# ShenhanQian/KGDet

Measured on AMD Instinct MI355X. Metric: training images/sec (whole node) KGDet R50-FPN 800x1333, higher is better.
Workload: dtype f32 (3 MFMA products per multiply on hi/lo-split operands -- fp16 parts forward, bf16 parts for gradients --, f32 accumulate); 1 GPU; KGDet R50-FPN train step, 2 img/GPU at 800x1333 (padded 800x1344), DeformConv fwd/bwd + focal/moment losses + grad-clip + Adam; no collective at dp1 (one rank: nothing to exchange); global_batch=2, parallelism=dp1

## Files before the change

### include/kgdet_hip.h

```cpp
#ifndef KGDET_HIP_H_
#define KGDET_HIP_H_

#include <stddef.h>
#include <stdint.h>

#ifdef __cplusplus
extern "C" {
#endif

#define KGDET_OK 0
#define KGDET_E_SHAPE 1
#define KGDET_E_WORKSPACE 2
#define KGDET_E_HIP 3
size_t kgdet_conv_packed_bytes(int32_t M, int32_t K, int32_t taps);
int kgdet_conv_pack(const float *w, int32_t O, int32_t C, int32_t taps, int32_t transpose, void *packed, void *stream);
int kgdet_conv_pack_fmt(const float *w, int32_t O, int32_t C, int32_t taps, int32_t transpose, void *packed,
                        int32_t operand_format, void *stream);
int kgdet_conv_pack_both_fmt(const float *w, int32_t O, int32_t C, int32_t taps, void *packed, void *packed_t,
                             int32_t forward_format, void *stream);
int kgdet_conv_apply_epilogue_fmt(const void *packed, const float *x, float *y, const float *bias, const float *residual,
                                  int32_t relu, int64_t B, int32_t M, int32_t K, int32_t H, int32_t W, int32_t taps,
                                  int32_t stride, int32_t operand_format, void *workspace, size_t workspace_bytes,
                                  void *stream);
int kgdet_conv_apply_gated_fmt(const void *packed, const float *x, float *y, const float *bias, const float *residual,
                               int32_t relu, const float *gate, int64_t B, int32_t M, int32_t K, int32_t H, int32_t W,
                               int32_t taps, int32_t stride, int32_t operand_format, void *workspace, size_t workspace_bytes,
                               void *stream);
int kgdet_stem_conv7x7_s2_fmt(const void *packed, const float *x, float *y, int64_t B, int32_t H, int32_t W,
                              int32_t operand_format, void *stream);
int kgdet_conv_pack_both(const float *w, int32_t O, int32_t C, int32_t taps, void *packed, void *packed_t, void *stream);
int64_t kgdet_conv_pack_blocks(int32_t O, int32_t C, int32_t taps);
int kgdet_conv_pack_multi(const int64_t *desc_dev, int32_t n, int64_t total_blocks, void *stream);
size_t kgdet_conv_apply_workspace_bytes(int64_t B, int32_t M, int32_t K, int32_t H, int32_t W, int32_t taps,
                                        int32_t stride);
int kgdet_conv_apply(const void *packed, const float *x, float *y, int64_t B, int32_t M, int32_t K, int32_t H, int32_t W,
                     int32_t taps, int32_t stride, void *workspace, size_t workspace_bytes, void *stream);
int kgdet_conv_apply_epilogue(const void *packed, const float *x, float *y, const float *bias, const float *residual,
                              int32_t relu, int64_t B, int32_t M, int32_t K, int32_t H, int32_t W, int32_t taps,
                              int32_t stride, void *workspace, size_t workspace_bytes, void *stream);
int kgdet_stem_conv7x7_s2(const void *packed, const float *x, float *y, int64_t B, int32_t H, int32_t W, void *stream);
int kgdet_conv3x3_s2_grad_input(const void *packed_t, const float *grad_y, float *grad_x, int64_t B, int32_t C, int32_t O,
                                int32_t Hin, int32_t Win, void *stream);
size_t kgdet_conv3x3_s2_grad_weight_workspace_bytes(int64_t B, int32_t O, int32_t C, int32_t H, int32_t W);
int kgdet_conv3x3_s2_grad_weight(const float *grad_y, const float *x, float *grad_w, int64_t B, int32_t O, int32_t C, int32_t H,
                                 int32_t W, void *workspace, size_t workspace_bytes, void *stream);
size_t kgdet_conv1x1_grad_weight_workspace_bytes(int64_t B, int32_t O, int32_t C, int64_t HW);
int kgdet_conv1x1_grad_weight(const float *grad_y, const float *x, float *grad_w, int64_t B, int32_t O, int32_t C,
                              int64_t HW, void *workspace, size_t workspace_bytes, void *stream);
size_t kgdet_conv3x3_grad_weight_workspace_bytes(int64_t B, int32_t O, int32_t C, int32_t H, int32_t W);
int kgdet_conv3x3_grad_weight(const float *grad_y, const float *x, float *grad_w, int64_t B, int32_t O, int32_t C,
                              int32_t H, int32_t W, void *workspace, size_t workspace_bytes, void *stream);

int kgdet_bn_act_forward(const float *x, const float *gamma, const float *beta, const float *mean, const float *var,
                         float eps, const float *residual, float *y, int64_t N, int32_t C, int64_t HW, int32_t relu,
                         void *stream);
int32_t kgdet_bn_act_partials(int64_t N, int32_t C, int64_t HW);
int kgdet_bn_act_backward(const float *grad_y, const float *x, const float *y, const float *gamma, const float *beta,
                          const float *mean, const float *var, float eps, int32_t has_residual, int32_t relu,
                          float *grad_x, float *grad_residual, float *partial, float *sums, int64_t N, int32_t C,
                          int64_t HW, void *stream);
int kgdet_conv1x1_nhwc_residual(const void *x, const void *weight, const float *bias, const void *residual, void *out,
                                int64_t M, int32_t K, int32_t N, int32_t relu, void *stream);
int kgdet_conv1x1_nhwc_residual_in(const void *x, const float *in_bias, const void *weight, const float *bias,
                                   const void *residual, void *out, int64_t M, int32_t K, int32_t N, int32_t relu,
                                   void *stream);
int kgdet_bn_fold_backward(const float *grad_z, const float *z, int32_t relu, float *g, float *partial, int64_t N, int32_t C,
                           int64_t HW, void *stream);
int kgdet_bn_fold_finish(const float *partial, int32_t P, const float *w, float *G , const float *s,
                         const float *mean, const float *var, float eps, float *grad_beta ,
                         float *grad_gamma , int32_t O, int32_t CK, void *stream);
int kgdet_conv1x1_grad_weight_fold(const float *grad_y, const float *x, float *grad_w, int64_t B, int32_t O, int32_t C,
                                   int64_t HW, void *workspace, size_t workspace_bytes, const float *w, const float *s,
                                   const float *mean, const float *var, float eps, const float *bn_partial, int32_t P,
                                   float *grad_beta , float *grad_gamma , void *stream);
int kgdet_conv3x3_grad_weight_fold(const float *grad_y, const float *x, float *grad_w, int64_t B, int32_t O, int32_t C,
                                   int32_t H, int32_t W, void *workspace, size_t workspace_bytes, const float *w,
                                   const float *s, const float *mean, const float *var, float eps, const float *bn_partial,
                                   int32_t P, float *grad_beta , float *grad_gamma , void *stream);
int kgdet_bn_relu_maxpool(const float *x, const float *gamma, const float *beta, const float *mean, const float *var,
                          float eps, float *y, int64_t N, int32_t C, int32_t H, int32_t W, void *stream);

int kgdet_bias_act(void *x, const float *bias, const void *residual, int64_t N, int32_t C, int64_t HW, int32_t dtype,
                   int32_t relu, int32_t channels_last, void *stream);
int kgdet_bias_relu_maxpool_nhwc(const void *x, const float *bias, void *y, int64_t N, int32_t C, int32_t H, int32_t W,
                                 int32_t dtype, void *stream);

#define KGDET_E_UNSUPPORTED 4
#define KGDET_E_PARTIAL 5

const char *kgdet_last_error(void);
int kgdet_version(void);
int kgdet_device_cu_count(void);

#define KGDET_OPT_EXACT_BACKWARD 0
#define KGDET_OPT_FWD_COLUMN_WAVE 1
#define KGDET_OPT_WGRAD_STREAMK 2
#define KGDET_OPT_BWD_PHASE 3
#define KGDET_OPT_COUNT 4
int kgdet_set_option(int32_t option, int32_t value);

typedef struct kgdet_dcn_shape {
  int32_t N, C, H, W;
  int32_t O, kh, kw;
  int32_t stride_h, stride_w, pad_h, pad_w, dil_h, dil_w;
  int32_t groups, deformable_groups;
  int32_t out_channel_offset, out_channels_total;
} kgdet_dcn_shape;

#define KGDET_DCN_RELU 1u
#define KGDET_DCN_BF16 2u
#define KGDET_DCN_EXACT_FP32 4u

int kgdet_dcn_output_size(const kgdet_dcn_shape *s, int32_t *Ho, int32_t *Wo);

size_t kgdet_dcn_packed_weight_bytes(const kgdet_dcn_shape *s);
size_t kgdet_dcn_workspace_bytes(const kgdet_dcn_shape *s);

int kgdet_dcn_pack_weight(const kgdet_dcn_shape *s, const float *weight, float *packed, void *stream);
int kgdet_dcn_pack_weight_multi(int32_t n, const kgdet_dcn_shape *const *shapes, const float *const *weights,
                                float *const *packeds, void *stream);
int kgdet_dcn_pack_weight_images(int32_t n, const kgdet_dcn_shape *const *shapes, const float *const *weights,
                                 float *const *packeds, uint32_t images, void *stream);
int32_t kgdet_dcn_split_path_complete(const kgdet_dcn_shape *shape);
int kgdet_dcn_unpack_weight_grad(const kgdet_dcn_shape *s, const float *packed, float *grad_weight,
                                 int accumulate, void *stream);

int kgdet_deform_conv_forward(const kgdet_dcn_shape *s, const float *input, const float *offset,
                              const float *mask , const float *packed_weight,
                              const float *bias , float *output, uint32_t flags,
                              void *workspace, size_t workspace_bytes, void *stream);

size_t kgdet_dcn_group_workspace_bytes(int32_t n, const kgdet_dcn_shape *const *shapes);

int kgdet_deform_conv_forward_grouped(int32_t n, const kgdet_dcn_shape *const *shapes, const float *const *inputs,
                                      const float *const *offsets, const float *const *masks ,
                                      const float *const *packed_weights, const float *const *biases ,
                                      float *const *outputs, uint32_t flags, void *workspace,
                                      size_t workspace_bytes, void *stream);

int kgdet_deform_conv_grad_input(const kgdet_dcn_shape *s, const float *offset, const float *mask ,
                                 const float *packed_weight, const float *grad_output, float *grad_input,
                                 uint32_t flags, void *workspace, size_t workspace_bytes, void *stream);

int kgdet_deform_conv_grad_offset(const kgdet_dcn_shape *s, const float *input, const float *offset,
                                  const float *packed_weight, const float *grad_output, float *grad_offset,
                                  uint32_t flags, void *workspace, size_t workspace_bytes, void *stream);

int kgdet_deform_conv_backward_input_grouped(int32_t n, const kgdet_dcn_shape *const *shapes, const float *const *inputs,
                                             const float *const *offsets, const float *const *packed_weights,
                                             const float *const *grad_outputs, float *const *grad_inputs,
                                             float *const *grad_offsets, void *workspace, size_t workspace_bytes,
// ... 188 lines not shown
```

### kgdet_amd/csrc/dense_forward.hip

```cpp
#include "dense_common.h"

namespace kgdet {

__global__ __launch_bounds__(256) void conv1x1_pack(const float *__restrict__ w, int O, int C, int T, int transpose,
                                                    unsigned char *__restrict__ img, unsigned char *__restrict__ img_t,
                                                    int f16_forward) {
  if (gridDim.y == 2) {
    transpose = blockIdx.y;
    img = blockIdx.y ? img_t : img;
  }
  const bool f16 = f16_forward && !transpose;
  f16_saturate_on();
  const int M = transpose ? C : O, K = transpose ? O : C;
  const int k16s = (K + kTK - 1) / kTK;
  const long long total = (long long)((M + kTM - 1) / kTM) * k16s * T * 2 * kTM;
  for (long long i = blockIdx.x * 256LL + threadIdx.x; i < total; i += gridDim.x * 256LL) {
    const int row = (int)(i % kTM);
    const int khalf = (int)((i / kTM) & 1);
    const long long st = i / (2 * kTM);
    const int t = (int)(st % T);
    const int k16 = (int)((st / T) % k16s), mt = (int)(st / ((long long)T * k16s));
    const int m = mt * kTM + row, k0 = k16 * kTK + khalf * 8;
    float v[8];
#pragma unroll
// ... 48 lines not shown
        const f32x4 u = src[q];
        r[4 * q] = u[0]; r[4 * q + 1] = u[1]; r[4 * q + 2] = u[2]; r[4 * q + 3] = u[3];
      }
      const float sc9 = (scale && m < M) ? scale[m] : 1.0f;
#pragma unroll
      for (int t = 0; t < 9; ++t) {
        float v[8];
#pragma unroll
        for (int j = 0; j < 8; ++j) v[j] = m < M ? r[j * 9 + t] * sc9 : 0.0f;
        bf16x8 hi8, lo8;
        if (f16_forward) {
#pragma unroll
          for (int j = 0; j < 8; ++j) v[j] *= kF16WeightScale;
          split8_t<true>(v, hi8, lo8);
        } else {
          split8(v, hi8, lo8);
        }
        unsigned char *dst = img + (s2 * 9 + t) * kStage + khalf * (kTM * 16) + row * 16;
        *reinterpret_cast<bf16x8 *>(dst) = hi8;
        *reinterpret_cast<bf16x8 *>(dst + kPart) = lo8;
      }
      continue;
    }
    if (i >= total) continue;
    const int row = (int)(i % kTM);
    const int khalf = (int)((i / kTM) & 1);
    const long long st = i / (2 * kTM);
    const int t = (int)(st % T);
    const int k16 = (int)((st / T) % k16s), mt = (int)(st / ((long long)T * k16s));
    const int m = mt * kTM + row, k0 = k16 * kTK + khalf * 8;
    float v[8];
#pragma unroll
    for (int j = 0; j < 8; ++j) {
      const long long o = transpose ? k0 + j : m, ch = transpose ? m : k0 + j;
      v[j] = (m < M && k0 + j < K) ? w[(o * C + ch) * T + (transpose ? T - 1 - t : t)] : 0.0f;
      if (scale && m < M && k0 + j < K) v[j] *= scale[o];
    }
    bf16x8 hi8, lo8;
    if (f16_forward && !transpose) {
#pragma unroll
      for (int j = 0; j < 8; ++j) v[j] *= kF16WeightScale;
      split8_t<true>(v, hi8, lo8);
    } else {
      split8(v, hi8, lo8);
    }
    unsigned char *dst = img + st * kStage + khalf * (kTM * 16) + row * 16;
    *reinterpret_cast<bf16x8 *>(dst) = hi8;
    *reinterpret_cast<bf16x8 *>(dst + kPart) = lo8;
  }
}

constexpr int kPF = 4;

template <int TAPS, int NW = 4, bool F16 = false>
__global__ __launch_bounds__(128 * NW) void conv_nn(const unsigned char *__restrict__ img,
                                                      const float *__restrict__ x, float *__restrict__ y, int M, int K,
                                                      int H, int W, int n_mt, int n_nt, int tiles, int ksplit,
                                                      long long part_stride, int Hin, int Win, int stride,
                                                      const float *__restrict__ bias,
                                                      const float *__restrict__ residual, int relu,
    const float *__restrict__ gate = nullptr) {
  constexpr int TN = 32 * NW, kPartB = 2 * TN * 16, kBuf = kStage + 2 * kPartB;
  __shared__ __attribute__((aligned(16))) unsigned char smem[2 * kBuf];
  if constexpr (F16) f16_saturate_on();
  const int unit = xcd_tile(blockIdx.x, tiles * ksplit);
  if (unit >= tiles * ksplit) return;
  const int part = unit % ksplit, tile = unit / ksplit;
  const int tid = threadIdx.x, lane = tid & 63, wave = tid >> 6, wm = wave & 1, wn = wave >> 1;
  const int n_local = tid % TN, kq = tid / TN;
  const int N = H * W;
  const int S = TAPS * ((K + kTK - 1) / kTK), per = (S + ksplit - 1) / ksplit;
  const int s_begin = part * per, s_end = max(s_begin, min(S, s_begin + per));
  const int stages = s_end - s_begin;
  struct Regs {
    f32x4 a;
    float v[4];
    unsigned live;
  };
  const int mt = tile % n_mt, nt = (tile / n_mt) % n_nt, b = tile / (n_mt * n_nt);
  const int n0 = nt * TN;
  const int p = min(n0 + n_local, N - 1);
  unsigned ok = 1u;
  if (TAPS == 9) {
    const int h = (p / W) * stride, w = (p - (p / W) * W) * stride;
    ok = 0u;
#pragma unroll
    for (int t = 0; t < 9; ++t) {
      const int hh = h + t / 3 - 1, ww = w + t % 3 - 1;
      ok |= (hh >= 0 && hh < Hin && ww >= 0 && ww < Win) ? (1u << t) : 0u;
    }
  }
  const int Nin = Hin * Win;
  const int pin = stride == 1 ? p : (p / W) * stride * Win + (p - (p / W) * W) * stride;
  const float *xb = x + (long long)b * K * Nin + pin;
  const unsigned char *ai = img + (long long)mt * S * kStage + (tid & 511) * 16;

  f32x16 acc[2];
#pragma unroll
  for (int i = 0; i < 2; ++i)
#pragma unroll
    for (int r = 0; r < 16; ++r) acc[i][r] = 0.0f;

  auto issue = [&](int s, Regs &R) {
    const int sc = s_begin + min(s, stages - 1);
    R.a = *reinterpret_cast<const f32x4 *>(ai + (long long)sc * kStage);
    const int c16 = sc / TAPS, t = sc - c16 * TAPS;
    int shift = 0;
    R.live = 1u;
    if (TAPS == 9) {
      R.live = (ok >> t) & 1u;
      shift = R.live ? (t / 3 - 1) * Win + (t % 3 - 1) : 0;
    }
    const float *xp = xb + (long long)(c16 * kTK + kq * 4) * Nin + shift;
    if (TAPS == 1 && (K & (kTK - 1)) && c16 == K / kTK) {
#pragma unroll
      for (int j = 0; j < 4; ++j) R.v[j] = xb[(long long)min(c16 * kTK + kq * 4 + j, K - 1) * Nin];
    } else {
#pragma unroll
      for (int j = 0; j < 4; ++j) R.v[j] = xp[(long long)j * Nin];
    }
  };
  auto commit = [&](int buf, const Regs &R) {
    unsigned char *As = smem + buf * kBuf, *Bs = As + kStage;
    *reinterpret_cast<f32x4 *>(As + (tid & 511) * 16) = R.a;
    uint2 hi, lo;
    split_pair_t<F16>(R.live ? R.v[0] : 0.0f, R.live ? R.v[1] : 0.0f, hi.x, lo.x);
    split_pair_t<F16>(R.live ? R.v[2] : 0.0f, R.live ? R.v[3] : 0.0f, hi.y, lo.y);
    unsigned char *dst = Bs + (kq >> 1) * (TN * 16) + n_local * 16 + (kq & 1) * 8;
    *reinterpret_cast<uint2 *>(dst) = hi;
    *reinterpret_cast<uint2 *>(dst + kPartB) = lo;
  };
  auto multiply = [&](int buf) {
    const unsigned char *A = smem + buf * kBuf + (lane >> 5) * (kTM * 16) + (wm * 64 + (lane & 31)) * 16;
    const unsigned char *Bp = smem + buf * kBuf + kStage + (lane >> 5) * (TN * 16) + (wn * 32 + (lane & 31)) * 16;
    bf16x8 a[2][2], bb[2];
#pragma unroll
    for (int pt = 0; pt < 2; ++pt) {
      a[pt][0] = *reinterpret_cast<const bf16x8 *>(A + pt * kPart);
      a[pt][1] = *reinterpret_cast<const bf16x8 *>(A + pt * kPart + 32 * 16);
      bb[pt] = *reinterpret_cast<const bf16x8 *>(Bp + pt * kPartB);
    }
#pragma unroll
    for (int mi = 0; mi < 2; ++mi) {
      acc[mi] = mfma_t<F16>(a[1][mi], bb[0], acc[mi]);
      acc[mi] = mfma_t<F16>(a[0][mi], bb[1], acc[mi]);
      acc[mi] = mfma_t<F16>(a[0][mi], bb[0], acc[mi]);
    }
  };
  {
    Regs R[kPF];
#pragma unroll
    for (int i = 0; i < kPF; ++i) issue(i, R[i]);
    commit(0, R[0]);
    const int full = stages / kPF * kPF;
    for (int s0 = 0; s0 < full; s0 += kPF) {
#pragma unroll
      for (int u = 0; u < kPF; ++u) {
        const int s = s0 + u;
        __syncthreads();
        issue(s + kPF, R[u]);
        multiply(s & 1);
        commit((s + 1) & 1, R[(u + 1) % kPF]);
      }
    }
#pragma unroll
    for (int u = 0; u < kPF - 1; ++u) {
      const int s = full + u;
      if (s < stages) {
        __syncthreads();
        multiply(s & 1);
        if (s + 1 < stages) commit((s + 1) & 1, R[u + 1]);
      }
    }
  }

  float *yb = y + (long long)part * part_stride + (long long)b * M * N;
  const int n = n0 + wn * 32 + (lane & 31);
  if constexpr (F16) {
#pragma unroll
    for (int mi = 0; mi < 2; ++mi)
#pragma unroll
      for (int r = 0; r < 16; ++r) acc[mi][r] *= 1.0f / kF16WeightScale;
  }
  if (bias || residual) {
    const int nc = min(n, N - 1);
    float add[2][16];
#pragma unroll
    for (int mi = 0; mi < 2; ++mi)
#pragma unroll
      for (int r = 0; r < 16; ++r) {
        const int m = min(mt * kTM + wm * 64 + mi * 32 + (r & 3) + 8 * (r >> 2) + 4 * (lane >> 5), M - 1);
        float v = bias ? bias[m] : 0.0f;
        if (residual) v += residual[((long long)b * M + m) * N + nc];
        add[mi][r] = v;
      }
#pragma unroll
    for (int mi = 0; mi < 2; ++mi)
#pragma unroll
      for (int r = 0; r < 16; ++r) acc[mi][r] += add[mi][r];
  }
  if (gate) {
    const int nc = min(n, N - 1);
    float gv[2][16];
#pragma unroll
    for (int mi = 0; mi < 2; ++mi)
#pragma unroll
      for (int r = 0; r < 16; ++r) {
        const int m = min(mt * kTM + wm * 64 + mi * 32 + (r & 3) + 8 * (r >> 2) + 4 * (lane >> 5), M - 1);
        gv[mi][r] = gate[((long long)b * M + m) * N + nc];
      }
#pragma unroll
    for (int mi = 0; mi < 2; ++mi)
#pragma unroll
      for (int r = 0; r < 16; ++r) acc[mi][r] = gv[mi][r] > 0.0f ? acc[mi][r] : 0.0f;
  }
#pragma unroll
  for (int mi = 0; mi < 2; ++mi)
#pragma unroll
    for (int r = 0; r < 16; ++r) {
      const int m = mt * kTM + wm * 64 + mi * 32 + (r & 3) + 8 * (r >> 2) + 4 * (lane >> 5);
      if (m < M && n < N) yb[(long long)m * N + n] = relu ? fmaxf(acc[mi][r], 0.0f) : acc[mi][r];
    }
}

constexpr int kPatchMax = 256;
constexpr int kPatchPart = 2 * kPatchMax * 16;
constexpr int kPatchBuf = 2 * kPatchPart;
template <int WAVES, int NB, bool F16 = false>
__global__ __launch_bounds__(64 * WAVES) void conv3x3_patch4(const unsigned char *__restrict__ img,
                                                             const float *__restrict__ x, float *__restrict__ y, int M,
                                                             int K, int H, int W, int n_mt, int tiles_x, int n_nt,
                                                             int tiles, int ksplit, long long part_stride, int TX, int TY,
                                                             const float *__restrict__ bias,
                                                             const float *__restrict__ residual, int relu,
    const float *__restrict__ gate = nullptr) {
  __shared__ __attribute__((aligned(16))) unsigned char smem[2 * kPatchBuf];
  if constexpr (F16) f16_saturate_on();
  constexpr int HALVES = 4 / WAVES, THREADS = 64 * WAVES, PXT = kPatchMax / THREADS;
  const int unit0 = xcd_tile(blockIdx.x, tiles * ksplit * HALVES);
  if (unit0 >= tiles * ksplit * HALVES) return;
  const int half = unit0 % HALVES, unit = unit0 / HALVES;
  const int part = unit % ksplit, tile = unit / ksplit;
  const int tid = threadIdx.x, lane = tid & 63, wave = (tid >> 6) + half * WAVES;
  const int N = H * W;
  const int chunks_all = K / kTK, per = (chunks_all + ksplit - 1) / ksplit;
  const int c_begin = part * per, c_end = max(c_begin, min(chunks_all, c_begin + per));
  const int chunks = c_end - c_begin, stages = chunks * 9;
  const int mt = tile % n_mt, nt = (tile / n_mt) % n_nt, b = tile / (n_mt * n_nt);
  const int y0 = (nt / tiles_x) * TY, x0 = (nt % tiles_x) * TX;
  const int PW = TX + 2, PP = PW * (TY + 2);

  if (mt * kTM + half * 64 >= M) return;
  bool p_live[PXT];
  int p_off[PXT];
#pragma unroll
  for (int i = 0; i < PXT; ++i) {
    const int pp = tid + i * THREADS;
    const int ppy = pp / PW, ppx = pp - ppy * PW;
    const int iy = y0 - 1 + ppy, ix = x0 - 1 + ppx;
    p_live[i] = pp < PP && iy >= 0 && iy < H && ix >= 0 && ix < W;
    p_off[i] = p_live[i] ? iy * W + ix : 0;
  }
  const float *xb = x + (long long)b * K * N;
  unsigned char *b_dst = smem + tid * 16;

  int b_rd[NB], o_n[NB];
  bool o_live[NB];
#pragma unroll
  for (int nb = 0; nb < NB; ++nb) {
    const int qq = nb * 32 + (lane & 31), q = min(qq, TX * TY - 1);
    const int py = q / TX, px = q - py * TX;
    b_rd[nb] = ((lane >> 5) * kPatchMax + py * PW + px) * 16;
    o_live[nb] = qq < TX * TY && y0 + py < H && x0 + px < W;
// ... 303 lines not shown

__global__ __launch_bounds__(256) void conv1x1_sum_epilogue(const float *__restrict__ parts, float *__restrict__ out,
                                                            long long n, long long stride, int count,
                                                            const float *__restrict__ bias, const float *__restrict__ residual,
                                                            int relu, int M, long long HW,
                                                            const float *__restrict__ gate = nullptr) {
  for (long long i = (blockIdx.x * 256LL + threadIdx.x) * 2; i < n; i += gridDim.x * 512LL) {
    f32x2 s = {0.0f, 0.0f};
    int k = 0;
    for (; k + 4 <= count; k += 4) {
      f32x2 v[4];
#pragma unroll
      for (int e = 0; e < 4; ++e) v[e] = *reinterpret_cast<const f32x2 *>(parts + (long long)(k + e) * stride + i);
#pragma unroll
      for (int e = 0; e < 4; ++e) s += v[e];
    }
    for (; k < count; ++k) s += *reinterpret_cast<const f32x2 *>(parts + (long long)k * stride + i);
    if (bias) {
      const float b = bias[(i / HW) % M];
      s[0] += b; s[1] += b;
    }
    if (residual) s += *reinterpret_cast<const f32x2 *>(residual + i);
    if (relu) { s[0] = fmaxf(s[0], 0.0f); s[1] = fmaxf(s[1], 0.0f); }
    if (gate) {
      const f32x2 gv = *reinterpret_cast<const f32x2 *>(gate + i);
      s[0] = gv[0] > 0.0f ? s[0] : 0.0f; s[1] = gv[1] > 0.0f ? s[1] : 0.0f;
    }
    *reinterpret_cast<f32x2 *>(out + i) = s;
  }
}

namespace {

long long pack_items(int M, int K, int taps) { return (long long)ceil_div(M, kTM) * ceil_div(K, kTK) * taps * 2 * kTM; }
long long pack_both_blocks(int O, int C, int taps) {
  const long long t0 = pack_items(O, C, taps), t1 = pack_items(C, O, taps);
  return ((t0 > t1 ? t0 : t1) + 255) / 256;
}

template <typename Kernel, typename... Args>
void launch_fmt(bool f16, Kernel bf16_kernel, Kernel f16_kernel, unsigned grid, unsigned block, void *stream, Args... args) {
  hipLaunchKernelGGL(f16 ? f16_kernel : bf16_kernel, dim3(grid), dim3(block), 0, (hipStream_t)stream, args...);
}

int nn_ksplit(long long tiles, int stages) {
  if (tiles >= 200) return 1;
  int k = (int)((384 + tiles - 1) / tiles);
  const int most = stages / 8;
  if (k > most) k = most;
  if (k > 8) k = 8;
  return k < 1 ? 1 : k;
}

struct NNPlan {
  bool patch;
  int TX, TY, NB, NW, tiles_x, n_nt, ks;
  long long tiles;
};
NNPlan plan_nn(long long B, int M, int K, int H, int W, int taps, int stride) {
  NNPlan p;
  const int Ho = (H + stride - 1) / stride, Wo = (W + stride - 1) / stride;
  const int n_mt = (M + kTM - 1) / kTM;
  p.patch = taps == 9 && stride == 1;
  p.TX = p.TY = p.tiles_x = 0;
  p.NB = p.NW = 4;
  p.n_nt = (int)(((long long)Ho * Wo + kTN - 1) / kTN);
  if (p.patch) {
    long long best = -1;
    for (int cap = 128; cap <= (M > 64 ? 160 : 128); cap += 32)
      for (int tx = 8; tx <= 126 && tx <= (W + 7) / 8 * 8; ++tx) {
        const int ty = cap / tx;
        if (ty < 1 || (tx + 2) * (ty + 2) > kPatchMax) continue;
        const long long n = (long long)((H + ty - 1) / ty) * ((W + tx - 1) / tx);
        const long long units = n * n_mt * B;
        const long long rounds = units <= 256 ? 256 : units <= 512 ? 512 : units;
        const long long cost = (rounds * (cap / 32)) * 4096 + n * 8 + (cap == 160) * 4 + ((tx + 2) * (ty + 2) > 230);
        if (best < 0 || cost < best) { best = cost; p.TX = tx; p.TY = ty; p.NB = cap / 32; }
      }
    static const int force_tx = env_int("KGDET_CONV_TX", 0);
    if (force_tx > 0 && (force_tx + 2) * (128 / force_tx + 2) <= kPatchMax) { p.TX = force_tx; p.TY = 128 / force_tx; p.NB = 4; }
    p.tiles_x = (W + p.TX - 1) / p.TX;
    p.n_nt = p.tiles_x * ((H + p.TY - 1) / p.TY);
  } else {
    static const int force_nw = env_int("KGDET_CONV_NW", 0);
    const long long hw = (long long)Ho * Wo;
    const long long u4 = (long long)n_mt * ((hw + 127) / 128) * B, u5 = (long long)n_mt * ((hw + 159) / 160) * B;
    const long long c4 = ((u4 + 255) / 256) * 4, c5 = ((u5 + 255) / 256) * 5;
    if (force_nw == 5 || (force_nw == 0 && u4 >= 200 && u5 >= 200 && c5 * 10 <= c4 * 9)) {
      p.NW = 5;
      p.n_nt = (int)((hw + 159) / 160);
    }
  }
  p.tiles = (long long)n_mt * p.n_nt * B;
  p.ks = nn_ksplit(p.tiles, taps * ((K + kTK - 1) / kTK));
  if (p.patch && p.tiles < 200) {
    const int chunks = K / kTK;
    double best = 1e30;
    p.ks = 1;
    for (int ks = 1; ks <= 8 && ks * 2 <= chunks; ++ks) {
      const double out_mb = (double)B * M * Ho * Wo * 4e-6;
      const double cost = (double)((p.tiles * ks + 255) / 256) * ((chunks + ks - 1) / ks) + 0.114 * out_mb * ks;
      if (cost < best) { best = cost; p.ks = ks; }
    }
  }
  static const int force_ks = env_int("KGDET_CONV_KS", 0);
  if (force_ks > 0) p.ks = force_ks;
  return p;
}

}

}

using namespace kgdet;

extern "C" size_t kgdet_conv_packed_bytes(int32_t M, int32_t K, int32_t taps) {
  if (M <= 0 || K <= 0 || (taps == 9 && K % kTK) || (taps != 1 && taps != 9)) return 0;
  return (size_t)pack_items(M, K, taps) * 32;
}

extern "C" int kgdet_conv_pack_fmt(const float *w, int32_t O, int32_t C, int32_t taps, int32_t transpose, void *packed,
                                   int32_t operand_format, void *stream) {
  const int M = transpose ? C : O, K = transpose ? O : C;
  KGDET_CHECK_SHAPE(taps == 1 || taps == 9, "taps must be 1 (1x1) or 9 (3x3)");
  KGDET_CHECK_SHAPE(O > 0 && C > 0 && (taps == 1 || K % kTK == 0), "reduction length %d is not a multiple of 16", K);
  KGDET_CHECK_SHAPE(w && packed, "null pointer");
  const long long blocks = (pack_items(M, K, taps) + 255) / 256;
  hipLaunchKernelGGL(conv1x1_pack, dim3((unsigned)(blocks > 65535 ? 65535 : blocks)), dim3(256), 0, (hipStream_t)stream, w,
                     O, C, taps, transpose, (unsigned char *)packed, (unsigned char *)nullptr, operand_format == 1 ? 1 : 0);
  KGDET_CHECK_LAUNCH("conv_pack");
  return KGDET_OK;
}

extern "C" int kgdet_conv_pack(const float *w, int32_t O, int32_t C, int32_t taps, int32_t transpose, void *packed,
                               void *stream) {
  return kgdet_conv_pack_fmt(w, O, C, taps, transpose, packed, 0, stream);
}

extern "C" int kgdet_conv_pack_both_fmt(const float *w, int32_t O, int32_t C, int32_t taps, void *packed, void *packed_t,
                                        int32_t forward_format, void *stream) {
  KGDET_CHECK_SHAPE(taps == 1 || taps == 9, "taps must be 1 (1x1) or 9 (3x3)");
  KGDET_CHECK_SHAPE(O > 0 && C > 0 && (taps == 1 || (O % kTK == 0 && C % kTK == 0)), "O and C must be multiples of 16");
  KGDET_CHECK_SHAPE(w && packed && packed_t, "null pointer");
  const long long blocks = pack_both_blocks(O, C, taps);
  hipLaunchKernelGGL(conv1x1_pack, dim3((unsigned)(blocks > 32768 ? 32768 : blocks), 2), dim3(256), 0,
                     (hipStream_t)stream, w, O, C, taps, 0, (unsigned char *)packed, (unsigned char *)packed_t,
                     forward_format == 1 ? 1 : 0);
  KGDET_CHECK_LAUNCH("conv_pack_both");
  return KGDET_OK;
}

extern "C" int kgdet_conv_pack_both(const float *w, int32_t O, int32_t C, int32_t taps, void *packed, void *packed_t,
                                    void *stream) {
  return kgdet_conv_pack_both_fmt(w, O, C, taps, packed, packed_t, 0, stream);
}

extern "C" int64_t kgdet_conv_pack_blocks(int32_t O, int32_t C, int32_t taps) {
  if (O <= 0 || C <= 0 || (taps == 9 && (O % kTK || C % kTK)) || (taps != 1 && taps != 9)) return 0;
  return pack_both_blocks(O, C, taps);
}

extern "C" int kgdet_conv_pack_multi(const int64_t *desc_dev, int32_t n, int64_t total_blocks, void *stream) {
  KGDET_CHECK_SHAPE(desc_dev && n > 0 && total_blocks > 0 && total_blocks < (1LL << 31), "bad descriptor table");
  hipLaunchKernelGGL(conv1x1_pack_multi, dim3((unsigned)total_blocks), dim3(256), 0, (hipStream_t)stream,
                     (const long long *)desc_dev, n);
  KGDET_CHECK_LAUNCH("conv_pack_multi");
  return KGDET_OK;
}

extern "C" size_t kgdet_conv_apply_workspace_bytes(int64_t B, int32_t M, int32_t K, int32_t H, int32_t W,
                                                    int32_t taps, int32_t stride) {
  if (B <= 0 || M <= 0 || K <= 0 || H <= 0 || W <= 0 || (taps == 9 && K % kTK) || stride < 1 || stride > 2) return 0;
  const long long HW = (long long)((H + stride - 1) / stride) * ((W + stride - 1) / stride);
  const int ks = plan_nn(B, M, K, H, W, taps, stride).ks;
  return ks > 1 ? (size_t)ks * B * M * HW * sizeof(float) : 0;
}

extern "C" int kgdet_conv_apply_epilogue_fmt(const void *packed, const float *x, float *y, const float *bias,
                                             const float *residual, int32_t relu, int64_t B, int32_t M, int32_t K,
                                             int32_t H, int32_t W, int32_t taps, int32_t stride, int32_t operand_format,
                                             void *workspace, size_t workspace_bytes, void *stream) {
  return kgdet_conv_apply_gated_fmt(packed, x, y, bias, residual, relu, nullptr, B, M, K, H, W, taps, stride, operand_format,
                                    workspace, workspace_bytes, stream);
}

extern "C" int kgdet_conv_apply_gated_fmt(const void *packed, const float *x, float *y, const float *bias,
                                          const float *residual, int32_t relu, const float *gate, int64_t B, int32_t M,
                                          int32_t K, int32_t H, int32_t W, int32_t taps, int32_t stride,
                                          int32_t operand_format, void *workspace, size_t workspace_bytes, void *stream) {
  const bool f16 = operand_format == 1;
  KGDET_CHECK_SHAPE(B >= 0 && M > 0 && K > 0 && H >= 0 && W >= 0 && (long long)H * W < (1LL << 30), "bad sizes");
  KGDET_CHECK_SHAPE(taps == 1 || taps == 9, "taps must be 1 (1x1) or 9 (3x3)");
  KGDET_CHECK_SHAPE(stride == 1 || stride == 2, "stride must be 1 or 2");
  KGDET_CHECK_SHAPE(taps == 1 || K % kTK == 0, "reduction length %d is not a multiple of 16", K);
  const int Ho = (H + stride - 1) / stride, Wo = (W + stride - 1) / stride;
  const long long HW = (long long)Ho * Wo;
  if (B * HW == 0) return KGDET_OK;
  KGDET_CHECK_SHAPE(packed && x && y, "null pointer");
  const NNPlan plan = plan_nn(B, M, K, H, W, taps, stride);
  const int n_mt = (M + kTM - 1) / kTM, n_nt = plan.n_nt;
  const long long tiles = plan.tiles;
  KGDET_CHECK_SHAPE(tiles < (1LL << 28), "too many tiles");
  const int ks = plan.ks;
  const long long part_stride = B * M * HW;
  if (ks > 1) {
    KGDET_CHECK_SHAPE(workspace && workspace_bytes >= (size_t)ks * part_stride * sizeof(float), "workspace too small");
    KGDET_CHECK_SHAPE(part_stride % 2 == 0, "B*M*Ho*Wo must be even");
    KGDET_CHECK_SHAPE(!gate || HW % 2 == 0, "a gated K-split convolution needs an even pixel count");
  }
  const unsigned grid = (unsigned)((tiles * ks + 7) / 8) * 8;
  float *dst = ks > 1 ? (float *)workspace : y;
  const float *k_bias = ks > 1 ? nullptr : bias, *k_residual = ks > 1 ? nullptr : residual, *k_gate = ks > 1 ? nullptr : gate;
  const int k_relu = ks > 1 ? 0 : relu;
  const unsigned char *img = (const unsigned char *)packed;
  if (plan.patch) {
    static const int force_halves = env_int("KGDET_CONV_HALVES", -1);
    const bool halves = force_halves >= 0 ? force_halves != 0 : ((ks == 1 && tiles > 256 && tiles < 400) || M <= 64);
    auto launch = [&](auto bf16_kernel, auto f16_kernel, unsigned g, unsigned threads) {
      launch_fmt(f16, bf16_kernel, f16_kernel, g, threads, stream, img, x, dst, M, K, H, W, n_mt, plan.tiles_x, n_nt, (int)tiles,
                 ks, part_stride, plan.TX, plan.TY, k_bias, k_residual, k_relu, k_gate);
    };
    if (plan.NB == 5)
      launch(conv3x3_patch4<4, 5, false>, conv3x3_patch4<4, 5, true>, grid, 256);
    else if (halves)
      launch(conv3x3_patch4<2, 4, false>, conv3x3_patch4<2, 4, true>, (unsigned)((tiles * ks * 2 + 7) / 8) * 8, 128);
    else
      launch(conv3x3_patch4<4, 4, false>, conv3x3_patch4<4, 4, true>, grid, 256);
  } else {
    auto launch = [&](auto bf16_kernel, auto f16_kernel, unsigned threads) {
      launch_fmt(f16, bf16_kernel, f16_kernel, grid, threads, stream, img, x, dst, M, K, Ho, Wo, n_mt, n_nt, (int)tiles, ks,
                 part_stride, H, W, stride, k_bias, k_residual, k_relu, k_gate);
    };
    if (taps == 1 && plan.NW == 5)
      launch(conv_nn<1, 5, false>, conv_nn<1, 5, true>, 640);
    else if (taps == 1)
      launch(conv_nn<1, 4, false>, conv_nn<1, 4, true>, 512);
    else if (plan.NW == 5)
      launch(conv_nn<9, 5, false>, conv_nn<9, 5, true>, 640);
    else
      launch(conv_nn<9, 4, false>, conv_nn<9, 4, true>, 512);
  }
  KGDET_CHECK_LAUNCH("conv_nn");
  if (ks > 1) {
    const long long blocks = (part_stride / 2 + 255) / 256;
    if ((bias || residual || relu || gate) && HW % 2 == 0)
      hipLaunchKernelGGL(conv1x1_sum_epilogue, dim3((unsigned)(blocks > 2048 ? 2048 : blocks)), dim3(256), 0,
                         (hipStream_t)stream, (const float *)workspace, y, part_stride, part_stride, ks, bias, residual, relu,
                         M, (long long)HW, gate);
    else
      hipLaunchKernelGGL(conv1x1_sum, dim3((unsigned)(blocks > 2048 ? 2048 : blocks)), dim3(256), 0, (hipStream_t)stream,
                         (const float *)workspace, y, part_stride, part_stride, ks);
    KGDET_CHECK_LAUNCH("conv1x1_sum");
    if ((bias || residual || relu) && HW % 2 != 0) return kgdet_bias_act(y, bias, residual, B, M, HW, 0, relu, 0, stream);
  }
  return KGDET_OK;
}

extern "C" int kgdet_conv_apply_epilogue(const void *packed, const float *x, float *y, const float *bias,
                                         const float *residual, int32_t relu, int64_t B, int32_t M, int32_t K,
                                         int32_t H, int32_t W, int32_t taps, int32_t stride, void *workspace,
                                         size_t workspace_bytes, void *stream) {
  return kgdet_conv_apply_epilogue_fmt(packed, x, y, bias, residual, relu, B, M, K, H, W, taps, stride, 0, workspace,
                                       workspace_bytes, stream);
}

extern "C" int kgdet_conv3x3_s2_grad_input(const void *packed_t, const float *grad_y, float *grad_x, int64_t B, int32_t C,
                                           int32_t O, int32_t Hin, int32_t Win, void *stream) {
  KGDET_CHECK_SHAPE(B >= 0 && C > 0 && O > 0 && Hin > 0 && Win > 0 && O % kTK == 0, "bad sizes (O must be a multiple of 16)");
  if (B == 0) return KGDET_OK;
  KGDET_CHECK_SHAPE(packed_t && grad_y && grad_x, "null pointer");
  const int H = (Hin + 1) / 2, W = (Win + 1) / 2;
  int TX = 0, TY = 0;
  long long best = -1;
  for (int tx = 8; tx <= 64; ++tx) {
    const int ty = 64 / tx;
    if (ty < 1 || (tx + 2) * (ty + 2) > kPatchMax) continue;
    const long long n = (long long)((H + ty - 1) / ty) * ((W + tx - 1) / tx);
    const long long cost = n * 1024 + (tx + 2) * (ty + 2);
    if (best < 0 || cost < best) { best = cost; TX = tx; TY = ty; }
  }
  const int n_mt = (C + kTM - 1) / kTM, tiles_x = (W + TX - 1) / TX, n_nt = tiles_x * ((H + TY - 1) / TY);
  const long long tiles = (long long)n_mt * n_nt * B;
  KGDET_CHECK_SHAPE(tiles < (1LL << 28), "too many tiles");
  hipLaunchKernelGGL(conv3x3_s2_grad_input, dim3((unsigned)((tiles + 7) / 8 * 8)), dim3(256), 0, (hipStream_t)stream,
                     (const unsigned char *)packed_t, grad_y, grad_x, C, O, H, W, Hin, Win, n_mt, tiles_x, n_nt, (int)tiles, TX, TY);
  KGDET_CHECK_LAUNCH("conv3x3_s2_grad_input");
// ... 29 lines not shown
```

Measured before the change: 186.4 img/s.

## Add 64-row conv_nn workgroups and cost-model choice of row tile and K-split

Templates the forward conv_nn kernel on a 64-row output tile, where four waves are laid out along the pixels. The planner gains an occupancy- and cost-based rule that picks 64-row tiles and a matching K-split for small tile counts (under 200 tiles), for both the generic and the patch 3x3 paths. The aim is to fill more of the 256 CUs on low-parallelism layers where 128-row tiles leave most CUs idle. In exchange the A operand is re-read per half-tile and the choice rests on hand-tuned constants. A plan query API and option knobs are also added.

```diff
diff --git a/include/kgdet_hip.h b/include/kgdet_hip.h
--- a/include/kgdet_hip.h
+++ b/include/kgdet_hip.h
@@ -33,6 +33,12 @@
 int kgdet_conv_pack_multi(const int64_t *desc_dev, int32_t n, int64_t total_blocks, void *stream);
 size_t kgdet_conv_apply_workspace_bytes(int64_t B, int32_t M, int32_t K, int32_t H, int32_t W, int32_t taps,
                                         int32_t stride);
+typedef struct kgdet_conv_plan {
+  int32_t rows, pixel_tile, tile_w, tile_h, ks, patch;
+  int64_t workgroups;
+} kgdet_conv_plan;
+int kgdet_conv_apply_plan(int64_t B, int32_t M, int32_t K, int32_t H, int32_t W, int32_t taps, int32_t stride,
+                          kgdet_conv_plan *plan);
 int kgdet_conv_apply(const void *packed, const float *x, float *y, int64_t B, int32_t M, int32_t K, int32_t H, int32_t W,
                      int32_t taps, int32_t stride, void *workspace, size_t workspace_bytes, void *stream);
 int kgdet_conv_apply_epilogue(const void *packed, const float *x, float *y, const float *bias, const float *residual,
@@ -96,7 +102,9 @@
 #define KGDET_OPT_FWD_COLUMN_WAVE 1
 #define KGDET_OPT_WGRAD_STREAMK 2
 #define KGDET_OPT_BWD_PHASE 3
-#define KGDET_OPT_COUNT 4
+#define KGDET_OPT_CONV_ROWS 4
+#define KGDET_OPT_CONV_KS 5
+#define KGDET_OPT_COUNT 6
 int kgdet_set_option(int32_t option, int32_t value);
 
 typedef struct kgdet_dcn_shape {
diff --git a/kgdet_amd/csrc/dense_forward.hip b/kgdet_amd/csrc/dense_forward.hip
--- a/kgdet_amd/csrc/dense_forward.hip
+++ b/kgdet_amd/csrc/dense_forward.hip
@@ -124,21 +124,28 @@
 
 constexpr int kPF = 4;
 
-template <int TAPS, int NW = 4, bool F16 = false>
-__global__ __launch_bounds__(128 * NW) void conv_nn(const unsigned char *__restrict__ img,
+constexpr int nn_threads(int rows, int nw) { return rows * nw; }
+constexpr int nn_lds_bytes(int rows, int nw) { return 2 * (rows * 64 + 2 * (2 * 32 * nw * 16)); }
+template <int TAPS, int NW = 4, bool F16 = false, int ROWS = 128>
+__global__ __launch_bounds__(nn_threads(ROWS, NW)) void conv_nn(const unsigned char *__restrict__ img,
                                                       const float *__restrict__ x, float *__restrict__ y, int M, int K,
                                                       int H, int W, int n_mt, int n_nt, int tiles, int ksplit,
                                                       long long part_stride, int Hin, int Win, int stride,
                                                       const float *__restrict__ bias,
                                                       const float *__restrict__ residual, int relu,
     const float *__restrict__ gate = nullptr) {
-  constexpr int TN = 32 * NW, kPartB = 2 * TN * 16, kBuf = kStage + 2 * kPartB;
+  static_assert(ROWS == 128 || (ROWS == 64 && NW == 4), "64-row workgroups: four waves along the pixels only");
+  constexpr int WM = ROWS / 64, THREADS = nn_threads(ROWS, NW);
+  constexpr int kPartA = 2 * ROWS * 16, kStageA = 2 * kPartA;
+  constexpr int TN = 32 * NW, kPartB = 2 * TN * 16, kBuf = kStageA + 2 * kPartB;
+  constexpr int CPT = kTK * TN / THREADS, QPT = CPT / 4;
+  static_assert(2 * kBuf == nn_lds_bytes(ROWS, NW), "plan_nn counts co-resident workgroups from nn_lds_bytes");
   __shared__ __attribute__((aligned(16))) unsigned char smem[2 * kBuf];
   if constexpr (F16) f16_saturate_on();
   const int unit = xcd_tile(blockIdx.x, tiles * ksplit);
   if (unit >= tiles * ksplit) return;
   const int part = unit % ksplit, tile = unit / ksplit;
-  const int tid = threadIdx.x, lane = tid & 63, wave = tid >> 6, wm = wave & 1, wn = wave >> 1;
+  const int tid = threadIdx.x, lane = tid & 63, wave = tid >> 6, wm = wave % WM, wn = wave / WM;
   const int n_local = tid % TN, kq = tid / TN;
   const int N = H * W;
   const int S = TAPS * ((K + kTK - 1) / kTK), per = (S + ksplit - 1) / ksplit;
@@ -146,10 +153,11 @@
   const int stages = s_end - s_begin;
   struct Regs {
     f32x4 a;
-    float v[4];
+    float v[CPT];
     unsigned live;
   };
   const int mt = tile % n_mt, nt = (tile / n_mt) % n_nt, b = tile / (n_mt * n_nt);
+  const int row0 = mt * ROWS;
   const int n0 = nt * TN;
   const int p = min(n0 + n_local, N - 1);
   unsigned ok = 1u;
@@ -165,7 +173,9 @@
   const int Nin = Hin * Win;
   const int pin = stride == 1 ? p : (p / W) * stride * Win + (p - (p / W) * W) * stride;
   const float *xb = x + (long long)b * K * Nin + pin;
-  const unsigned char *ai = img + (long long)mt * S * kStage + (tid & 511) * 16;
+  const int a_src = ROWS == 128 ? (tid & 511) * 16 : (tid >> 6) * (kTM * 16) + ((mt & 1) * 64 + (tid & 63)) * 16;
+  const int a_dst = ROWS == 128 ? (tid & 511) * 16 : tid * 16;
+  const unsigned char *ai = img + (long long)(row0 / kTM) * S * kStage + a_src;
 
   f32x16 acc[2];
 #pragma unroll
@@ -183,33 +193,37 @@
       R.live = (ok >> t) & 1u;
       shift = R.live ? (t / 3 - 1) * Win + (t % 3 - 1) : 0;
     }
-    const float *xp = xb + (long long)(c16 * kTK + kq * 4) * Nin + shift;
+    const float *xp = xb + (long long)(c16 * kTK + kq * CPT) * Nin + shift;
     if (TAPS == 1 && (K & (kTK - 1)) && c16 == K / kTK) {
 #pragma unroll
-      for (int j = 0; j < 4; ++j) R.v[j] = xb[(long long)min(c16 * kTK + kq * 4 + j, K - 1) * Nin];
+      for (int j = 0; j < CPT; ++j) R.v[j] = xb[(long long)min(c16 * kTK + kq * CPT + j, K - 1) * Nin];
     } else {
 #pragma unroll
-      for (int j = 0; j < 4; ++j) R.v[j] = xp[(long long)j * Nin];
+      for (int j = 0; j < CPT; ++j) R.v[j] = xp[(long long)j * Nin];
     }
   };
   auto commit = [&](int buf, const Regs &R) {
-    unsigned char *As = smem + buf * kBuf, *Bs = As + kStage;
-    *reinterpret_cast<f32x4 *>(As + (tid & 511) * 16) = R.a;
-    uint2 hi, lo;
-    split_pair_t<F16>(R.live ? R.v[0] : 0.0f, R.live ? R.v[1] : 0.0f, hi.x, lo.x);
-    split_pair_t<F16>(R.live ? R.v[2] : 0.0f, R.live ? R.v[3] : 0.0f, hi.y, lo.y);
-    unsigned char *dst = Bs + (kq >> 1) * (TN * 16) + n_local * 16 + (kq & 1) * 8;
-    *reinterpret_cast<uint2 *>(dst) = hi;
-    *reinterpret_cast<uint2 *>(dst + kPartB) = lo;
+    unsigned char *As = smem + buf * kBuf, *Bs = As + kStageA;
+    *reinterpret_cast<f32x4 *>(As + a_dst) = R.a;
+#pragma unroll
+    for (int q = 0; q < QPT; ++q) {
+      const int g = kq * QPT + q;
+      uint2 hi, lo;
+      split_pair_t<F16>(R.live ? R.v[4 * q] : 0.0f, R.live ? R.v[4 * q + 1] : 0.0f, hi.x, lo.x);
+      split_pair_t<F16>(R.live ? R.v[4 * q + 2] : 0.0f, R.live ? R.v[4 * q + 3] : 0.0f, hi.y, lo.y);
+      unsigned char *dst = Bs + (g >> 1) * (TN * 16) + n_local * 16 + (g & 1) * 8;
+      *reinterpret_cast<uint2 *>(dst) = hi;
+      *reinterpret_cast<uint2 *>(dst + kPartB) = lo;
+    }
   };
   auto multiply = [&](int buf) {
-    const unsigned char *A = smem + buf * kBuf + (lane >> 5) * (kTM * 16) + (wm * 64 + (lane & 31)) * 16;
-    const unsigned char *Bp = smem + buf * kBuf + kStage + (lane >> 5) * (TN * 16) + (wn * 32 + (lane & 31)) * 16;
+    const unsigned char *A = smem + buf * kBuf + (lane >> 5) * (ROWS * 16) + (wm * 64 + (lane & 31)) * 16;
+    const unsigned char *Bp = smem + buf * kBuf + kStageA + (lane >> 5) * (TN * 16) + (wn * 32 + (lane & 31)) * 16;
     bf16x8 a[2][2], bb[2];
 #pragma unroll
     for (int pt = 0; pt < 2; ++pt) {
-      a[pt][0] = *reinterpret_cast<const bf16x8 *>(A + pt * kPart);
-      a[pt][1] = *reinterpret_cast<const bf16x8 *>(A + pt * kPart + 32 * 16);
+      a[pt][0] = *reinterpret_cast<const bf16x8 *>(A + pt * kPartA);
+      a[pt][1] = *reinterpret_cast<const bf16x8 *>(A + pt * kPartA + 32 * 16);
       bb[pt] = *reinterpret_cast<const bf16x8 *>(Bp + pt * kPartB);
     }
 #pragma unroll
@@ -261,7 +275,7 @@
     for (int mi = 0; mi < 2; ++mi)
 #pragma unroll
       for (int r = 0; r < 16; ++r) {
-        const int m = min(mt * kTM + wm * 64 + mi * 32 + (r & 3) + 8 * (r >> 2) + 4 * (lane >> 5), M - 1);
+        const int m = min(row0 + wm * 64 + mi * 32 + (r & 3) + 8 * (r >> 2) + 4 * (lane >> 5), M - 1);
         float v = bias ? bias[m] : 0.0f;
         if (residual) v += residual[((long long)b * M + m) * N + nc];
         add[mi][r] = v;
@@ -278,7 +292,7 @@
     for (int mi = 0; mi < 2; ++mi)
 #pragma unroll
       for (int r = 0; r < 16; ++r) {
-        const int m = min(mt * kTM + wm * 64 + mi * 32 + (r & 3) + 8 * (r >> 2) + 4 * (lane >> 5), M - 1);
+        const int m = min(row0 + wm * 64 + mi * 32 + (r & 3) + 8 * (r >> 2) + 4 * (lane >> 5), M - 1);
         gv[mi][r] = gate[((long long)b * M + m) * N + nc];
       }
 #pragma unroll
@@ -290,7 +304,7 @@
   for (int mi = 0; mi < 2; ++mi)
 #pragma unroll
     for (int r = 0; r < 16; ++r) {
-      const int m = mt * kTM + wm * 64 + mi * 32 + (r & 3) + 8 * (r >> 2) + 4 * (lane >> 5);
+      const int m = row0 + wm * 64 + mi * 32 + (r & 3) + 8 * (r >> 2) + 4 * (lane >> 5);
       if (m < M && n < N) yb[(long long)m * N + n] = relu ? fmaxf(acc[mi][r], 0.0f) : acc[mi][r];
     }
 }
@@ -700,59 +714,135 @@
   return k < 1 ? 1 : k;
 }
 
+constexpr int kCUs = 256, kLdsPerCU = 160 * 1024, kSimds = 4, kWaveSlots = 8, kRegsPerSimd = 512;
+constexpr int resident(int lds_bytes, int waves, int registers) {
+  const int by_lds = kLdsPerCU / lds_bytes, by_slots = kWaveSlots * kSimds / waves;
+  const int by_regs = kRegsPerSimd / registers * kSimds / waves;
+  const int r = by_lds < by_slots ? by_lds : by_slots;
+  return r < by_regs ? r : by_regs;
+}
+constexpr int kNN64Resident = resident(nn_lds_bytes(64, 4), nn_threads(64, 4) / 64, 136);
+constexpr int kPatch64Resident = resident(2 * kPatchBuf, 2, 200);
+static_assert(kNN64Resident == 3 && kPatch64Resident == 4, "see the row rule's constants");
+
+constexpr double kNNAlone64 = 0.99, kNNShared64 = 0.63, kNNFixed = 13.5, kNNSum = 8.25, kNNPartialPerMB = 0.63;
+constexpr double kPatchAlone64 = 0.90, kPatchShared64 = 0.70, kPatchSum = 1.0, kPatchPartialPerMB = 0.114;
+constexpr double kRows64Margin = 0.90;
+
+double rows64_time(long long units, int resident_wgs, double alone, double shared) {
+  const long long c = (units + kCUs - 1) / kCUs;
+  const double a = alone * (double)((c + resident_wgs - 1) / resident_wgs), b = shared * (double)c;
+  return a > b ? a : b;
+}
+
 struct NNPlan {
   bool patch;
-  int TX, TY, NB, NW, tiles_x, n_nt, ks;
+  int rows, TX, TY, NB, NW, tiles_x, n_nt, ks;
   long long tiles;
+  long long workgroups;
 };
 NNPlan plan_nn(long long B, int M, int K, int H, int W, int taps, int stride) {
   NNPlan p;
   const int Ho = (H + stride - 1) / stride, Wo = (W + stride - 1) / stride;
-  const int n_mt = (M + kTM - 1) / kTM;
+  const int n_mt = (M + kTM - 1) / kTM, n_mt64 = (M + 63) / 64;
+  static const int env_rows = env_int("KGDET_CONV_ROWS", 0);
+  const int force_rows = g_options[KGDET_OPT_CONV_ROWS] ? g_options[KGDET_OPT_CONV_ROWS] : env_rows;
+  static const int env_ks = env_int("KGDET_CONV_KS", 0);
+  const int force_ks = g_options[KGDET_OPT_CONV_KS] > 0 ? g_options[KGDET_OPT_CONV_KS] : env_ks;
   p.patch = taps == 9 && stride == 1;
+  p.rows = 128;
   p.TX = p.TY = p.tiles_x = 0;
   p.NB = p.NW = 4;
   p.n_nt = (int)(((long long)Ho * Wo + kTN - 1) / kTN);
+  const double out_mb = (double)B * M * Ho * Wo * 4e-6;
   if (p.patch) {
-    long long best = -1;
-    for (int cap = 128; cap <= (M > 64 ? 160 : 128); cap += 32)
-      for (int tx = 8; tx <= 126 && tx <= (W + 7) / 8 * 8; ++tx) {
-        const int ty = cap / tx;
-        if (ty < 1 || (tx + 2) * (ty + 2) > kPatchMax) continue;
-        const long long n = (long long)((H + ty - 1) / ty) * ((W + tx - 1) / tx);
-        const long long units = n * n_mt * B;
-        const long long rounds = units <= 256 ? 256 : units <= 512 ? 512 : units;
-        const long long cost = (rounds * (cap / 32)) * 4096 + n * 8 + (cap == 160) * 4 + ((tx + 2) * (ty + 2) > 230);
-        if (best < 0 || cost < best) { best = cost; p.TX = tx; p.TY = ty; p.NB = cap / 32; }
-      }
-    static const int force_tx = env_int("KGDET_CONV_TX", 0);
-    if (force_tx > 0 && (force_tx + 2) * (128 / force_tx + 2) <= kPatchMax) { p.TX = force_tx; p.TY = 128 / force_tx; p.NB = 4; }
-    p.tiles_x = (W + p.TX - 1) / p.TX;
-    p.n_nt = p.tiles_x * ((H + p.TY - 1) / p.TY);
-  } else {
-    static const int force_nw = env_int("KGDET_CONV_NW", 0);
-    const long long hw = (long long)Ho * Wo;
-    const long long u4 = (long long)n_mt * ((hw + 127) / 128) * B, u5 = (long long)n_mt * ((hw + 159) / 160) * B;
-    const long long c4 = ((u4 + 255) / 256) * 4, c5 = ((u5 + 255) / 256) * 5;
-    if (force_nw == 5 || (force_nw == 0 && u4 >= 200 && u5 >= 200 && c5 * 10 <= c4 * 9)) {
-      p.NW = 5;
-      p.n_nt = (int)((hw + 159) / 160);
-    }
-  }
-  p.tiles = (long long)n_mt * p.n_nt * B;
-  p.ks = nn_ksplit(p.tiles, taps * ((K + kTK - 1) / kTK));
-  if (p.patch && p.tiles < 200) {
+    auto tile_shape = [&](int cap_max) {
+      long long best = -1;
+      for (int cap = 128; cap <= cap_max; cap += 32)
+        for (int tx = 8; tx <= 126 && tx <= (W + 7) / 8 * 8; ++tx) {
+          const int ty = cap / tx;
+          if (ty < 1 || (tx + 2) * (ty + 2) > kPatchMax) continue;
+          const long long n = (long long)((H + ty - 1) / ty) * ((W + tx - 1) / tx);
+          const long long units = n * n_mt * B;
+          const long long rounds = units <= 256 ? 256 : units <= 512 ? 512 : units;
+          const long long cost = (rounds * (cap / 32)) * 4096 + n * 8 + (cap == 160) * 4 + ((tx + 2) * (ty + 2) > 230);
+          if (best < 0 || cost < best) { best = cost; p.TX = tx; p.TY = ty; p.NB = cap / 32; }
+        }
+      static const int force_tx = env_int("KGDET_CONV_TX", 0);
+      if (force_tx > 0 && (force_tx + 2) * (128 / force_tx + 2) <= kPatchMax) { p.TX = force_tx; p.TY = 128 / force_tx; p.NB = 4; }
+      p.tiles_x = (W + p.TX - 1) / p.TX;
+      p.n_nt = p.tiles_x * ((H + p.TY - 1) / p.TY);
+      p.tiles = (long long)n_mt * p.n_nt * B;
+    };
     const int chunks = K / kTK;
+    auto best_split = [&](int rows, double *cost_out) {
+      double best = 1e30;
+      int best_ks = 1;
+      for (int ks = 1; ks <= 8 && (ks == 1 || ks * 2 <= chunks); ++ks) {
+        const int per = (chunks + ks - 1) / ks;
+        double cost = rows == 128 ? (double)((p.tiles * ks + 255) / 256) * per + kPatchPartialPerMB * out_mb * ks
+                                  : rows64_time((long long)n_mt64 * p.n_nt * B * ks, kPatch64Resident, kPatchAlone64, kPatchShared64) * per +
+                                        (ks > 1 ? kPatchSum + kPatchPartialPerMB * out_mb * ks : 0.0);
+        if (force_ks > 0 && ks != force_ks) continue;
+        if (cost < best) { best = cost; best_ks = ks; }
+      }
+      if (cost_out) *cost_out = rows == 64 ? best : best + (best_ks > 1 ? kPatchSum : -kPatchPartialPerMB * out_mb);
+      return force_ks > 0 ? force_ks : best_ks;
+    };
+    static const int force_halves = env_int("KGDET_CONV_HALVES", -1);
+    const int want_rows = force_rows == 64 || force_rows == 128 ? force_rows : force_halves >= 0 ? (force_halves ? 64 : 128) : 0;
+    tile_shape(M > 64 && want_rows != 64 ? 160 : 128);
+    p.ks = 1;
+    if (p.tiles < 200) p.ks = best_split(128, nullptr);
+    if (force_ks > 0) p.ks = force_ks;
+    bool halves = p.NB == 4 && ((p.ks == 1 && p.tiles > 256 && p.tiles < 400) || M <= 64);
+    if (want_rows) halves = want_rows == 64 && p.NB == 4;
+    if (!want_rows && !halves && p.tiles < 200 && M > 64) {
+      const NNPlan whole = p;
+      double c128, c64;
+      best_split(128, &c128);
+      tile_shape(128);
+      const int ks64 = best_split(64, &c64);
+      if (c64 < kRows64Margin * c128) { halves = true; p.ks = ks64; } else { p = whole; }
+    }
+    p.rows = halves ? 64 : 128;
+    p.workgroups = p.tiles * p.ks * (halves ? 2 : 1);
+    return p;
+  }
+  static const int force_nw = env_int("KGDET_CONV_NW", 0);
+  const long long hw = (long long)Ho * Wo;
+  const long long u4 = (long long)n_mt * ((hw + 127) / 128) * B, u5 = (long long)n_mt * ((hw + 159) / 160) * B;
+  const long long c4 = ((u4 + 255) / 256) * 4, c5 = ((u5 + 255) / 256) * 5;
+  if (force_rows != 64 && (force_nw == 5 || (force_nw == 0 && u4 >= 200 && u5 >= 200 && c5 * 10 <= c4 * 9))) {
+    p.NW = 5;
+    p.n_nt = (int)((hw + 159) / 160);
+  }
+  const int S = taps * ((K + kTK - 1) / kTK);
+  const long long tiles128 = (long long)n_mt * p.n_nt * B, tiles64 = (long long)n_mt64 * p.n_nt * B;
+  p.tiles = tiles128;
+  p.ks = nn_ksplit(p.tiles, S);
+  if (force_rows == 64) p.rows = 64;
+  if (force_rows == 0 && tiles128 < 200 && p.NW == 4) {
+    auto cost = [&](int rows, int ks) {
+      const int per = (S + ks - 1) / ks;
+      const double t = rows == 128 ? (double)((tiles128 * ks + kCUs - 1) / kCUs)
+                                   : rows64_time(tiles64 * ks, kNN64Resident, kNNAlone64, kNNShared64);
+      return t * (per + kNNFixed) + (ks > 1 ? kNNSum + kNNPartialPerMB * out_mb * ks : 0.0);
+    };
+    const int ks128 = force_ks > 0 ? force_ks : p.ks;
+    const double c128 = cost(128, ks128);
     double best = 1e30;
-    p.ks = 1;
-    for (int ks = 1; ks <= 8 && ks * 2 <= chunks; ++ks) {
-      const double out_mb = (double)B * M * Ho * Wo * 4e-6;
-      const double cost = (double)((p.tiles * ks + 255) / 256) * ((chunks + ks - 1) / ks) + 0.114 * out_mb * ks;
-      if (cost < best) { best = cost; p.ks = ks; }
-    }
-  }
-  static const int force_ks = env_int("KGDET_CONV_KS", 0);
+    int ks64 = 1;
+    for (int ks = 1; ks <= ks128 && (ks == 1 || ks * 8 <= S); ++ks) {
+      if ((force_ks > 0 && ks != force_ks) || ks == 5 || ks == 7) continue;
+      const double c = cost(64, ks);
+      if (c < best) { best = c; ks64 = ks; }
+    }
+    if (best < kRows64Margin * c128) { p.rows = 64; p.ks = ks64; }
+  }
   if (force_ks > 0) p.ks = force_ks;
+  if (p.rows == 64) p.tiles = tiles64;
+  p.workgroups = p.tiles * p.ks;
   return p;
 }
 
@@ -822,6 +912,22 @@
   const long long HW = (long long)((H + stride - 1) / stride) * ((W + stride - 1) / stride);
   const int ks = plan_nn(B, M, K, H, W, taps, stride).ks;
   return ks > 1 ? (size_t)ks * B * M * HW * sizeof(float) : 0;
+}
+
+extern "C" int kgdet_conv_apply_plan(int64_t B, int32_t M, int32_t K, int32_t H, int32_t W, int32_t taps, int32_t stride,
+                                     kgdet_conv_plan *plan) {
+  KGDET_CHECK_SHAPE(plan, "null pointer");
+  KGDET_CHECK_SHAPE(B > 0 && M > 0 && K > 0 && H > 0 && W > 0 && (taps == 1 || (taps == 9 && K % kTK == 0)) &&
+                        (stride == 1 || stride == 2), "bad sizes");
+  const NNPlan p = plan_nn(B, M, K, H, W, taps, stride);
+  plan->rows = p.rows;
+  plan->pixel_tile = p.patch ? 32 * p.NB : 32 * p.NW;
+  plan->tile_w = p.patch ? p.TX : 0;
+  plan->tile_h = p.patch ? p.TY : 0;
+  plan->ks = p.ks;
+  plan->patch = p.patch ? 1 : 0;
+  plan->workgroups = p.workgroups;
+  return KGDET_OK;
 }
 
 extern "C" int kgdet_conv_apply_epilogue_fmt(const void *packed, const float *x, float *y, const float *bias,
@@ -862,8 +968,7 @@
   const int k_relu = ks > 1 ? 0 : relu;
   const unsigned char *img = (const unsigned char *)packed;
   if (plan.patch) {
-    static const int force_halves = env_int("KGDET_CONV_HALVES", -1);
-    const bool halves = force_halves >= 0 ? force_halves != 0 : ((ks == 1 && tiles > 256 && tiles < 400) || M <= 64);
+    const bool halves = plan.rows == 64;
     auto launch = [&](auto bf16_kernel, auto f16_kernel, unsigned g, unsigned threads) {
       launch_fmt(f16, bf16_kernel, f16_kernel, g, threads, stream, img, x, dst, M, K, H, W, n_mt, plan.tiles_x, n_nt, (int)tiles,
                  ks, part_stride, plan.TX, plan.TY, k_bias, k_residual, k_relu, k_gate);
@@ -875,11 +980,16 @@
     else
       launch(conv3x3_patch4<4, 4, false>, conv3x3_patch4<4, 4, true>, grid, 256);
   } else {
+    const int n_rt = (M + plan.rows - 1) / plan.rows;
     auto launch = [&](auto bf16_kernel, auto f16_kernel, unsigned threads) {
-      launch_fmt(f16, bf16_kernel, f16_kernel, grid, threads, stream, img, x, dst, M, K, Ho, Wo, n_mt, n_nt, (int)tiles, ks,
+      launch_fmt(f16, bf16_kernel, f16_kernel, grid, threads, stream, img, x, dst, M, K, Ho, Wo, n_rt, n_nt, (int)tiles, ks,
                  part_stride, H, W, stride, k_bias, k_residual, k_relu, k_gate);
     };
-    if (taps == 1 && plan.NW == 5)
+    if (plan.rows == 64 && taps == 1)
+      launch(conv_nn<1, 4, false, 64>, conv_nn<1, 4, true, 64>, 256);
+    else if (plan.rows == 64)
+      launch(conv_nn<9, 4, false, 64>, conv_nn<9, 4, true, 64>, 256);
+    else if (taps == 1 && plan.NW == 5)
       launch(conv_nn<1, 5, false>, conv_nn<1, 5, true>, 640);
     else if (taps == 1)
       launch(conv_nn<1, 4, false>, conv_nn<1, 4, true>, 512);
```

After: 185.3 img/s, median of 2. Within noise of the previous version (-0.6%).
